# acmater/prograph

Measured on NVIDIA B200. Metric: Gpairs/s Hamming all-pairs + kNN graph build, N=1M L=256, higher is better.
Workload: dtype u8 tokens -> 5 bit planes, int32 popcount distances

## Files before the change

prograph_b200/csrc/pg_sweep.cu:

```cuda
#include <vector>
#include <mutex>

#include <cub/device/device_scan.cuh>
#include <cub/device/device_select.cuh>
#include <cub/device/device_radix_sort.cuh>
#include <thrust/iterator/counting_iterator.h>

#include <cstdlib>
#include <cmath>

#include <algorithm>

#include "pg_sweep.cuh"
#include "pg_sweep_sym.cuh"

namespace pg {

static std::mutex g_time_mu;
static bool g_time_enabled = false;
static std::vector<std::pair<cudaEvent_t, cudaEvent_t>> g_time_events;

struct SweepTimer {
  cudaEvent_t a = nullptr, b = nullptr;
  cudaStream_t s;
// ... 216 lines not shown
        const unsigned long long e = __ldcs(src + j);
        out_idx[at + j] = static_cast<long long>(e & 0xffffffffull);
        write_weight(out_w, at + j, static_cast<int>(e >> 32), weight);
      }
      at += c;
    }
  }
}

static size_t eps_counts_bytes(const Geometry& g, long long rows) { return static_cast<size_t>(g.n_splits) * rows * 8; }
static size_t eps_capture_bytes(const Geometry& g, long long rows, int cap = kEpsCapture) {
  return static_cast<size_t>(g.n_splits) * rows * static_cast<size_t>(cap) * 8;
}
static size_t eps_flag_bytes(long long rows) { return static_cast<size_t>(round_up(rows, 256)); }
static size_t eps_list_bytes(long long rows) { return static_cast<size_t>(rows) * 8; }
constexpr int kEpsCaptureMax = 1 << 20;
constexpr size_t kEpsCaptureLimit = 8ull << 30;

struct EpsPlan {
  Geometry g;
  int cap;
};
static EpsPlan eps_plan(long long rows, long long stream_rows, int words, int capture) {
  EpsPlan p;
  p.cap = 0;
  if (capture > 0 && rows < (1ll << 31)) {
    const int cap = std::min(std::max(capture, kEpsCapture), kEpsCaptureMax);
    const long long splits = static_cast<long long>(kEpsCaptureLimit / (static_cast<size_t>(rows) * cap * 8));
    if (splits >= 1) {
      p.g = make_geometry(rows, stream_rows, words, kConsumers, 0, splits);
      p.cap = cap;
      return p;
    }
  }
  p.g = make_geometry(rows, stream_rows, words, kConsumers, 0);
  if (eps_capture_bytes(p.g, rows) <= kEpsCaptureLimit && rows < (1ll << 31)) p.cap = kEpsCapture;
  return p;
}
static size_t eps_plan_bytes(const EpsPlan& p, long long rows) {
  size_t bytes = eps_counts_bytes(p.g, rows) + 256;
  if (p.cap > 0) bytes += eps_flag_bytes(rows) + eps_list_bytes(rows) + eps_capture_bytes(p.g, rows, p.cap);
  return bytes;
}


static int dispatch_sym(int planes, int words, const SymParams& prm, const SymLaunch& l, int* resident) {
#define PG_CASE(P, W) \
  if (planes == P && words == W) return sweep_sym_p##P##_w##W(prm, l, resident);
  PG_CASE(5, 1) PG_CASE(5, 2) PG_CASE(5, 4) PG_CASE(5, 8) PG_CASE(5, 16)
  PG_CASE(8, 1) PG_CASE(8, 2) PG_CASE(8, 4) PG_CASE(8, 8)
#undef PG_CASE
  set_error("symmetric sweep supports planes in {5,8} x words in {1,2,4,8} and planes=5, words=16; got planes=%d "
            "words=%d", planes, words);
  return PG_ERR_UNSUPPORTED;
}

static bool sym_shape_ok(int planes, int words) {
  return ((planes == 5 || planes == 8) && (words == 1 || words == 2 || words == 4 || words == 8)) ||
         (planes == 5 && words == 16);
}

struct SymLayout {
  int tile_cols, n_tiles, n_blocks, band_tiles, n_bands;
  size_t gnt_bytes, lock_bytes, stats_off, item_off, item_bytes_max, total;
};

static int sym_band_tiles(int tile_cols, int row_bytes) {
  double mb = 24.0;
  if (const char* ev = std::getenv("PG_SYM_BAND_MB")) mb = std::atof(ev);
  if (mb <= 0) return 1 << 30;
  long long t = static_cast<long long>(mb * 1048576.0 / (static_cast<double>(tile_cols) * row_bytes));
  if (t < 64) t = 64;
  return static_cast<int>(std::min<long long>(t, 1 << 30));
}

static SymLayout sym_layout(long long rows, int words, int planes = 5) {
  SymLayout s;
  s.tile_cols = tile_cols_for(words);
  s.n_tiles = static_cast<int>(ceil_div(rows, s.tile_cols));
  s.n_blocks = static_cast<int>(ceil_div(rows, kConsumers));
  s.band_tiles = sym_band_tiles(s.tile_cols, planes * words * 4);
  s.n_bands = static_cast<int>(ceil_div(s.n_tiles, s.band_tiles));
  s.gnt_bytes = static_cast<size_t>(round_up(static_cast<int64_t>(s.n_tiles) * s.tile_cols * 8, 256));
  s.lock_bytes = static_cast<size_t>(round_up(rows * 4, 256));
  s.stats_off = s.gnt_bytes + s.lock_bytes;
  s.item_off = s.stats_off + 256;
  const int bands8 = static_cast<int>(ceil_div(s.n_tiles, sym_band_tiles(s.tile_cols, 8 * words * 4)));
  s.item_bytes_max = (static_cast<size_t>(s.n_blocks) * (2 * static_cast<size_t>(bands8) + 2) + 64ull * 4 * 160 + 1024) *
                         sizeof(SymItem) + 8192;
  s.total = s.item_off + s.item_bytes_max;
  return s;
}

static int sym_first_tile(const SymLayout& s, int rb, long long boot_rows) {
  const long long row = static_cast<long long>(rb) * kConsumers < boot_rows ? boot_rows
                                                                            : static_cast<long long>(rb) * kConsumers;
  return static_cast<int>(row / s.tile_cols);
}

static void sym_band(const SymLayout& s, long long rows, long long boot_rows, int part, int parts, int* t0, int* t1) {
  std::vector<long long> visits(static_cast<size_t>(s.n_tiles) + 1, 0);
  for (int rb = 0; rb < s.n_blocks; ++rb) {
    const int tb = sym_first_tile(s, rb, boot_rows);
    if (tb >= s.n_tiles) continue;
    const long long in_block = std::min<long long>(kConsumers, rows - static_cast<long long>(rb) * kConsumers);
    visits[tb] += in_block;
  }
  long long total = 0, run = 0;
  for (int t = 0; t < s.n_tiles; ++t) { run += visits[t]; visits[t] = run; total += run; }
  auto bound = [&](int g) {
    if (g <= 0) return 0;
    if (g >= parts) return s.n_tiles;
    const long long want = static_cast<long long>(static_cast<double>(total) * g / parts);
    long long acc = 0;
    for (int t = 0; t < s.n_tiles; ++t) {
      acc += visits[t];
      if (acc >= want) return t + 1;
    }
    return s.n_tiles;
  };
  *t0 = bound(part);
  *t1 = bound(part + 1);
}

struct SymPlan {
  std::vector<SymItem> items;
  std::vector<int> first;
  int grid = 0;
};

static SymPlan sym_plan(const SymLayout& s, long long rows, int part, int parts, int mode, int grid,
                        long long boot_rows, int chunk_floor = 32) {
  const int boot_blocks = static_cast<int>(boot_rows / kConsumers);
  int band0 = 0, band1 = s.n_tiles;
  if (mode == 1) sym_band(s, rows, boot_rows, part, parts, &band0, &band1);
  const int rb_first = mode == 1 ? 0 : part, rb_stride = mode == 1 ? 1 : parts;
  long long total = 0;
  for (int rb = rb_first; rb < s.n_blocks; rb += rb_stride)
// ... 19 lines not shown
      const int boot = rb < boot_blocks ? 1 : 0;
      const double g = (n_seen + 0.37 * sb) * 0.6180339887498949;
      const double frac = g - static_cast<long long>(g);
      int t = tb;
      const int first = static_cast<int>(chunk / 4 + static_cast<long long>(frac * static_cast<double>(chunk))) + 1;
      while (t < te) {
        int t1 = t + (t == tb ? first : static_cast<int>(chunk));
        if (te - t1 < chunk / 4) t1 = te;
        if (t1 > te) t1 = te;
        items.push_back(SymItem{rb, t, t1, boot});
        t = t1;
      }
    }
    std::stable_sort(items.begin(), items.end(),
                     [](const SymItem& a, const SymItem& b) { return a.t1 - a.t0 > b.t1 - b.t0; });
    for (int b = 0; b < grid; ++b) heap[b] = b;
    std::make_heap(heap.begin(), heap.end(), heavier);
    for (const SymItem& it : items) {
      std::pop_heap(heap.begin(), heap.end(), heavier);
      const int b = heap.back();
      per_cta[b].push_back(it);
      load[b] += (it.t1 - it.t0) + 4;
      std::push_heap(heap.begin(), heap.end(), heavier);
    }
  }
  SymPlan plan;
  plan.first.push_back(0);
  for (int b = 0; b < grid; ++b) {
    if (per_cta[b].empty()) continue;
    plan.items.insert(plan.items.end(), per_cta[b].begin(), per_cta[b].end());
    plan.first.push_back(static_cast<int>(plan.items.size()));
  }
  plan.grid = static_cast<int>(plan.first.size()) - 1;
  return plan;
}

static int sym_knn_chunk_floor(int words, int parts) { return (parts == 1 ? 256 : 32) * std::max(1, 8 / words); }

static size_t sym_plan_bytes(const SymPlan& p) {
  return static_cast<size_t>(round_up(static_cast<int64_t>(p.first.size()) * 4, 16)) + p.items.size() * sizeof(SymItem);
}
static int sym_upload_plan(const SymPlan& p, const SymLayout& lay, char* wsb, SymParams* prm, cudaStream_t cs) {
  PG_CHECK_ARG(sym_plan_bytes(p) <= lay.item_bytes_max, "item table overflow (%zu items)", p.items.size());
  const size_t first_bytes = static_cast<size_t>(round_up(static_cast<int64_t>(p.first.size()) * 4, 16));
  PG_CUDA(cudaMemcpyAsync(wsb + lay.item_off, p.first.data(), p.first.size() * 4, cudaMemcpyHostToDevice, cs));
  PG_CUDA(cudaMemcpyAsync(wsb + lay.item_off + first_bytes, p.items.data(), p.items.size() * sizeof(SymItem),
                          cudaMemcpyHostToDevice, cs));
  prm->cta_first = reinterpret_cast<const int*>(wsb + lay.item_off);
  prm->items = reinterpret_cast<const SymItem*>(wsb + lay.item_off + first_bytes);
  prm->n_items = static_cast<int>(p.items.size());
  return PG_OK;
}

__global__ void sym_init_kernel(unsigned long long* glist, long long n_keys, unsigned long long* glast, long long n_gnt, unsigned* glock,
                                long long rows, unsigned long long* stats, int k1, int seeded) {
  if (blockIdx.x == 0 && threadIdx.x < 9) stats[threadIdx.x] = 0ull;
  const long long i = blockIdx.x * static_cast<long long>(blockDim.x) + threadIdx.x;
  const long long stride = static_cast<long long>(gridDim.x) * blockDim.x;
  if (!seeded)
    for (long long j = i; j < n_keys; j += stride) glist[j] = ~0ull;
  for (long long j = i; j < n_gnt; j += stride) {
    unsigned long long last = ~0ull;
    if (seeded && j < rows) last = glist[j * k1 + (k1 - 1)];
    glast[j] = sym_filter_word(last);
  }
  for (long long j = i; j < rows; j += stride) glock[j] = 0u;
}

__global__ void knn_part_to_lists_kernel(const unsigned long long* __restrict__ part, int n_splits, int k1,
                                         long long rows, unsigned long long* __restrict__ lists) {
  extern __shared__ unsigned long long merge_sm[];
  const long long row_base = blockIdx.x * static_cast<long long>(blockDim.x);
  const long long r = row_base + threadIdx.x;
  unsigned long long* mine = merge_sm + threadIdx.x * (k1 + 1);
  if (r < rows) {
    unsigned long long last = 0;
    bool ended = false;
    for (int j = 0; j < k1; ++j) {
      unsigned long long best = ~0ull;
      if (!ended) {
        for (int s = 0; s < n_splits; ++s) {
          const unsigned long long* lst = part + static_cast<size_t>(s) * k1 * rows + r;
          for (int i = 0; i < k1; ++i) {
            const unsigned long long v = lst[static_cast<size_t>(i) * rows];
            if (j > 0 && v <= last) continue;
            if (v < best) best = v;
            break;
          }
        }
      }
      last = best;
      ended |= best == ~0ull;
      mine[j] = best;
    }
  }
  flush_rows(merge_sm, row_base, rows, k1, PG_W_I64, true, lists, nullptr, nullptr);
}

constexpr int kMaxMergeLists = 16;

__global__ void knn_lists_finalize_kernel(const unsigned long long* __restrict__ lists, int n_lists,
                                          long long list_stride, long long row0, long long rows, int k1, int k,
                                          int drop, int weight, bool keys_out, unsigned long long* __restrict__ out_keys,
                                          long long* __restrict__ out_idx, void* out_w) {
  extern __shared__ unsigned long long merge_sm[];
  const long long row_base = blockIdx.x * static_cast<long long>(blockDim.x);
  const long long r = row_base + threadIdx.x;
  unsigned long long* mine = merge_sm + threadIdx.x * (k + 1);
  if (r < rows) {
    const unsigned long long* base = lists + static_cast<size_t>(row0 + r) * k1;
    unsigned long long head[kMaxMergeLists];
    int pos[kMaxMergeLists];
#pragma unroll
    for (int s = 0; s < kMaxMergeLists; ++s) {
      pos[s] = 0;
      head[s] = s < n_lists ? base[static_cast<size_t>(s) * list_stride] : ~0ull;
    }
    for (int j = 0; j < drop + k; ++j) {
      unsigned long long best = ~0ull;
// ... 359 lines not shown
  }
  if (rc != PG_OK) return rc;
  const int threads = rows_per_merge_block(k1);
  knn_part_to_lists_kernel<<<static_cast<unsigned>(ceil_div(rows, threads)), threads, merge_smem_bytes(k1), l.stream>>>(
      prm.part, g.n_splits, k1, rows, reinterpret_cast<unsigned long long*>(lists));
  PG_LAUNCH_CHECK();
  return PG_OK;
}

int pg_knn_sym_band(int64_t rows, int words, int64_t boot_rows, int part, int parts, int64_t* row_begin,
                    int64_t* row_end) {
  PG_CHECK_ARG(rows > 0 && words > 0 && parts >= 1 && part >= 0 && part < parts && row_begin && row_end,
               "bad band arguments");
  const SymLayout lay = sym_layout(rows, words);
  int t0 = 0, t1 = 0;
  sym_band(lay, rows, boot_rows, part, parts, &t0, &t1);
  *row_begin = std::min<int64_t>(rows, static_cast<int64_t>(t0) * lay.tile_cols);
  *row_end = std::min<int64_t>(rows, static_cast<int64_t>(t1) * lay.tile_cols);
  return PG_OK;
}

int pg_knn_sym_plan(int64_t rows, int planes, int words, int64_t boot_rows, int part, int parts, int mode, int grid,
                    int32_t* items_host, int64_t capacity, int64_t* n_items) {
  PG_CHECK_ARG(rows > 0 && words > 0 && planes > 0 && parts >= 1 && part >= 0 && part < parts && grid >= 1 && n_items &&
                   (mode == 0 || mode == 1) && boot_rows >= 0 && boot_rows % kStreamRowPad == 0,
               "bad plan arguments");
  const SymLayout lay = sym_layout(rows, words, planes);
  const SymPlan plan = sym_plan(lay, rows, part, parts, mode, grid, boot_rows, sym_knn_chunk_floor(words, parts));
  *n_items = static_cast<int64_t>(plan.items.size());
  PG_CHECK_ARG(sym_plan_bytes(plan) <= lay.item_bytes_max, "item table overflow (%zu items)", plan.items.size());
  if (items_host) {
    int cta = 0;
    for (size_t i = 0; i < plan.items.size() && static_cast<int64_t>(i) < capacity; ++i) {
      while (static_cast<int>(i) >= plan.first[cta + 1]) ++cta;
      items_host[5 * i + 0] = plan.items[i].rb;
      items_host[5 * i + 1] = plan.items[i].t0;
      items_host[5 * i + 2] = plan.items[i].t1;
      items_host[5 * i + 3] = plan.items[i].boot;
      items_host[5 * i + 4] = cta;
    }
  }
  return PG_OK;
}

int pg_knn_sym_status(const void* workspace, int64_t rows, int words, void* stream) {
  PG_CHECK_ARG(workspace && rows > 0 && words > 0, "bad status arguments");
  const SymLayout lay = sym_layout(rows, words);
  unsigned err = 0;
  cudaStream_t cs = static_cast<cudaStream_t>(stream);
  PG_CUDA(cudaMemcpyAsync(&err, static_cast<const char*>(workspace) + lay.stats_off + 64, sizeof(err),
                          cudaMemcpyDeviceToHost, cs));
  PG_CUDA(cudaStreamSynchronize(cs));
  if (err != 0) {
    set_error("symmetric sweep: a row lock could not be taken within %u attempts (lists are incomplete)", kLockSpinLimit);
    return PG_ERR_CUDA;
  }
  return PG_OK;
}

int pg_hamming_knn_sym(const uint32_t* table, int64_t rows, int planes, int words, int k1, int part, int parts,
                       int mode, int64_t boot_rows, uint64_t* lists, void* workspace, size_t workspace_bytes,
                       void* stream) {
  const int rb_first = part, rb_stride = parts;
  PG_CHECK_ARG(mode == 0 || mode == 1, "bad partition mode %d", mode);
  PG_CHECK_ARG(table && lists && workspace, "null pointer");
  PG_CHECK_ARG(rows > 0 && rows < (1ll << 31), "row count out of range");
  PG_CHECK_ARG((reinterpret_cast<uintptr_t>(table) & 15) == 0, "table must be 16-byte aligned");
  PG_CHECK_ARG((reinterpret_cast<uintptr_t>(workspace) & 255) == 0, "workspace must be 256-byte aligned");
  PG_CHECK_ARG(rb_stride >= 1 && rb_first >= 0 && rb_first < rb_stride, "bad row-block interleave %d/%d", rb_first,
               rb_stride);
  PG_CHECK_ARG(boot_rows >= 0 && boot_rows % kStreamRowPad == 0 && boot_rows <= rows,
               "bootstrap rows must be a multiple of %d within the table", kStreamRowPad);
  if (!sym_shape_ok(planes, words) || k1 < 1 || k1 > 32) {
    set_error("symmetric sweep: planes/words %d/%d or list length %d not covered", planes, words, k1);
    return PG_ERR_UNSUPPORTED;
  }
  const SymLayout lay = sym_layout(rows, words, planes);
  PG_CHECK_ARG(workspace_bytes >= lay.total, "workspace too small: %zu < %zu", workspace_bytes, lay.total);
  cudaStream_t cs = static_cast<cudaStream_t>(stream);
  char* wsb = static_cast<char*>(workspace);
  SymParams prm;
  memset(&prm, 0, sizeof(prm));
  prm.tab = table;
  prm.rows = rows;
  prm.one = 1u;
  prm.k1 = k1;
  prm.boot_rows = boot_rows;
  prm.glist = reinterpret_cast<unsigned long long*>(lists);
  prm.glast = reinterpret_cast<unsigned long long*>(wsb);
  prm.glock = reinterpret_cast<unsigned*>(wsb + lay.gnt_bytes);
  unsigned long long* stats_dev = reinterpret_cast<unsigned long long*>(wsb + lay.stats_off);
  const bool want_stats = std::getenv("PG_SYM_STATS") != nullptr;
  prm.stats = want_stats ? stats_dev : nullptr;
  prm.error = reinterpret_cast<unsigned*>(stats_dev + 8);
  SymLaunch l{0, static_cast<size_t>(k1) * kConsumers * 8, cs, SYM_KNN};
  int resident = 0;
  int rc = dispatch_sym(planes, words, prm, l, &resident);
  if (rc != PG_OK) return rc;
  const SymPlan plan = sym_plan(lay, rows, part, parts, mode, resident, boot_rows, sym_knn_chunk_floor(words, parts));
  sym_init_kernel<<<num_sms() * 4, 256, 0, cs>>>(prm.glist, static_cast<long long>(rows) * k1, prm.glast,
                                                 static_cast<long long>(lay.n_tiles) * lay.tile_cols, prm.glock, rows,
                                                 stats_dev, k1, boot_rows > 0 ? 1 : 0);
  PG_LAUNCH_CHECK();
  if (plan.items.empty()) return PG_OK;
  rc = sym_upload_plan(plan, lay, wsb, &prm, cs);
  if (rc != PG_OK) return rc;
  l.grid = plan.grid;
  {
    SweepTimer t(cs);
    rc = dispatch_sym(planes, words, prm, l, nullptr);
  }
  if (rc == PG_OK && want_stats) {
    unsigned long long st[8];
    PG_CUDA(cudaMemcpyAsync(st, stats_dev, sizeof(st), cudaMemcpyDeviceToHost, cs));
    PG_CUDA(cudaStreamSynchronize(cs));
    fprintf(stderr, "[pg sym] rows=%lld boot=%lld items=%d grid=%d | locks %llu, lock spins %llu, list writes %llu | row "
            "inserts %llu\n", static_cast<long long>(rows), static_cast<long long>(boot_rows), prm.n_items, l.grid,
            st[1], st[2], st[3], st[4]);
  }
  return rc;
}

int pg_hamming_eps_sym(const uint32_t* table, int64_t rows, int planes, int words, const uint32_t* lut_host,
                       int lut_words, int part, int parts, int mode, uint64_t* keys, int64_t capacity,
                       uint64_t* counters, void* workspace, size_t workspace_bytes, void* stream) {
  PG_CHECK_ARG(table && keys && counters && workspace && lut_host, "null pointer");
  PG_CHECK_ARG(rows > 0 && rows < (1ll << 27), "row count out of range for packed edge keys");
  PG_CHECK_ARG((reinterpret_cast<uintptr_t>(table) & 15) == 0, "table must be 16-byte aligned");
  PG_CHECK_ARG((reinterpret_cast<uintptr_t>(workspace) & 255) == 0, "workspace must be 256-byte aligned");
  PG_CHECK_ARG(parts >= 1 && part >= 0 && part < parts && (mode == 0 || mode == 1), "bad partition %d/%d mode %d", part,
               parts, mode);
  PG_CHECK_ARG(lut_words >= 1 && lut_words <= kMaxLutWords && lut_words * 32 > words * 32, "lut must cover distances 0..%d",
               words * 32);
  PG_CHECK_ARG(capacity >= 0, "negative capacity");
  if (!sym_shape_ok(planes, words)) {
    set_error("symmetric sweep: planes/words %d/%d not covered", planes, words);
    return PG_ERR_UNSUPPORTED;
  }
  SymParams prm;
  memset(&prm, 0, sizeof(prm));
  unsigned span = 0;
  if (!lut_as_range(lut_host, lut_words, &prm.lo, &span)) {
    set_error("symmetric epsilon sweep needs a contiguous distance range");
    return PG_ERR_UNSUPPORTED;
  }
  prm.hi = prm.lo == 0x7fffffff ? -1 : prm.lo + static_cast<int>(span);
  if (prm.lo == 0x7fffffff) prm.lo = 1 << 20;
  const SymLayout lay = sym_layout(rows, words, planes);
  PG_CHECK_ARG(workspace_bytes >= lay.total, "workspace too small: %zu < %zu", workspace_bytes, lay.total);
  const EdgeKeyBits kb = edge_key_bits(rows, words);
  cudaStream_t cs = static_cast<cudaStream_t>(stream);
  char* wsb = static_cast<char*>(workspace);
  prm.tab = table;
  prm.rows = rows;
  prm.one = 1u;
  prm.k1 = 1;
  prm.sh_col = kb.dbits;
  prm.sh_row = kb.dbits + kb.idxbits;
  prm.keys = reinterpret_cast<unsigned long long*>(keys);
  prm.capacity = capacity;
  prm.counters = reinterpret_cast<unsigned long long*>(counters);
  SymLaunch l{0, 0, cs, SYM_EPS};
  int resident = 0;
  int rc = dispatch_sym(planes, words, prm, l, &resident);
  if (rc != PG_OK) return rc;
  const SymPlan plan = sym_plan(lay, rows, part, parts, mode, resident, 0);
  PG_CUDA(cudaMemsetAsync(counters, 0, 2 * sizeof(uint64_t), cs));
  if (plan.items.empty()) return PG_OK;
  rc = sym_upload_plan(plan, lay, wsb, &prm, cs);
// ... 148 lines not shown
```

prograph_b200/csrc/pg_sweep_inst.cu:

```cuda
#include "pg_sweep.cuh"
#include "pg_sweep_sym.cuh"

#ifndef PG_P
#error "compile with -DPG_P=<planes> -DPG_W=<words>"
#endif

#define PG_CAT2(a, b, c, d) a##b##c##d
#define PG_NAME(P, W) PG_CAT2(sweep_p, P, _w, W)

namespace pg {
int PG_NAME(PG_P, PG_W)(const SweepParams& prm, const SweepLaunch& l) { return launch_sweep<PG_P, PG_W>(prm, l); }
#define PG_SYM_NAME(P, W) PG_CAT2(sweep_sym_p, P, _w, W)
int PG_SYM_NAME(PG_P, PG_W)(const SymParams& prm, const SymLaunch& l, int* resident) {
  return launch_sweep_sym<PG_P, PG_W>(prm, l, resident);
}
}
```

prograph_b200/csrc/pg_sweep_sym.cuh:

```cuda
#pragma once
#include "pg_sweep.cuh"

namespace pg {

constexpr int kTauInf = 0x3fffffff;

struct SymItem { int rb, t0, t1, boot; };

struct SymParams {
  const uint32_t* tab;
  long long rows;
  const SymItem* items;
  const int* cta_first;
  int n_items;
  unsigned one;
  int k1;
  unsigned long long* glist;
  unsigned long long* glast;
  unsigned* glock;
  unsigned long long* stats;
  unsigned* error;
  long long boot_rows;
  int lo, hi;
  int sh_row, sh_col;
  unsigned long long* keys;
  long long capacity;
  unsigned long long* counters;
};

__device__ __forceinline__ unsigned long long ld_cg_u64(const unsigned long long* p) {
  unsigned long long v;
  asm volatile("ld.global.cg.u64 %0, [%1];" : "=l"(v) : "l"(p) : "memory");
  return v;
}
__device__ __forceinline__ void st_cg_u64(unsigned long long* p, unsigned long long v) {
  asm volatile("st.global.cg.u64 [%0], %1;" ::"l"(p), "l"(v) : "memory");
}
__device__ __forceinline__ unsigned atom_cas_acquire_gpu(unsigned* p, unsigned cmp, unsigned val) {
  unsigned old;
  asm volatile("atom.acquire.gpu.global.cas.b32 %0, [%1], %2, %3;" : "=r"(old) : "l"(p), "r"(cmp), "r"(val) : "memory");
  return old;
}
__device__ __forceinline__ void st_release_gpu_u32(unsigned* p, unsigned v) {
  asm volatile("st.release.gpu.global.u32 [%0], %1;" ::"l"(p), "r"(v) : "memory");
}
constexpr unsigned kLockSpinLimit = 1u << 24;
__host__ __device__ __forceinline__ unsigned long long sym_filter_word(unsigned long long last) {
  const unsigned tau = (last == ~0ull) ? static_cast<unsigned>(kTauInf) : static_cast<unsigned>(last >> 32);
  return (static_cast<unsigned long long>(~tau) << 32) | (last & 0xffffffffull);
}
__device__ __forceinline__ int mad_s32(int a, unsigned b, int c) {
  int r;
  asm("mad.lo.s32 %0, %1, %2, %3;" : "=r"(r) : "r"(a), "r"(b), "r"(c));
  return r;
}

static __device__ __noinline__ void sym_serve_col(const SymParams& prm, long long j, unsigned long long key, bool is_cand,
                                           int lane) {
  const int k1 = prm.k1;
  unsigned long long* lst = prm.glist + static_cast<size_t>(j) * k1;
  unsigned cand = __ballot_sync(0xffffffffu, is_cand);
  if (cand == 0u) return;
  unsigned* lock = prm.glock + j;
  unsigned got = 1u;
  if (lane == 0) {
    unsigned spins = 0;
    while (atom_cas_acquire_gpu(lock, 0u, 1u) != 0u) {
      __nanosleep(100);
      if (++spins > kLockSpinLimit) {
        got = 0u;
        atomicExch(prm.error, 1u);
        break;
      }
    }
    if (prm.stats != nullptr) {
      atomicAdd(prm.stats + 1, 1ull);
      if (spins) atomicAdd(prm.stats + 2, static_cast<unsigned long long>(spins));
    }
  }
  if (__shfl_sync(0xffffffffu, got, 0) == 0u) return;
  __syncwarp();
  unsigned long long e = lane < k1 ? ld_cg_u64(lst + lane) : ~0ull;
  bool changed = false;
  while (cand) {
    const int src = __ffs(cand) - 1;
    cand &= cand - 1;
    const unsigned long long kk = __shfl_sync(0xffffffffu, key, src);
    const int pos = __popc(__ballot_sync(0xffffffffu, lane < k1 && e < kk));
    const unsigned long long up = __shfl_up_sync(0xffffffffu, e, 1);
    if (pos < k1) {
      if (lane == pos) e = kk;
      else if (lane > pos) e = up;
      changed = true;
    }
  }
  if (changed) {
    if (lane < k1) st_cg_u64(lst + lane, e);
    const unsigned long long last = __shfl_sync(0xffffffffu, e, k1 - 1);
    if (lane == 0) {
      st_cg_u64(prm.glast + j, sym_filter_word(last));
      if (prm.stats != nullptr) atomicAdd(prm.stats + 3, 1ull);
    }
  }
  __syncwarp();
  if (lane == 0) st_release_gpu_u32(lock, 0u);
}

constexpr int kMaxSymList = 32;

static __device__ __noinline__ int sym_serve_row(unsigned long long* warp_lists, int k1, unsigned cand, unsigned dv,
                                          unsigned col, int lane, int tau_seed, int tau,
                                          unsigned long long* stats) {
  if (stats != nullptr && lane == 0) atomicAdd(stats + 4, static_cast<unsigned long long>(__popc(cand)));
  while (cand) {
    const int src = __ffs(cand) - 1;
    cand &= cand - 1;
    const unsigned dd = __shfl_sync(0xffffffffu, dv, src);
    const unsigned long long key = (static_cast<unsigned long long>(dd) << 32) | col;
    const unsigned t_new = knn_insert_coop(warp_lists + static_cast<size_t>(src) * k1, k1, key, lane);
    if (lane == src) tau = min(tau_seed, t_new == 0xffffffffu ? kTauInf : static_cast<int>(t_new));
  }
  return tau;
}

struct SymCursor {
  int idx, end, t, t1;
  __device__ __forceinline__ void start(int i, const SymParams& prm) {
    idx = i;
    if (idx < end) {
      const int4 it = __ldg(reinterpret_cast<const int4*>(prm.items) + idx);
      t = it.y;
      t1 = it.z;
    } else {
      t = t1 = 0;
    }
  }
  __device__ __forceinline__ bool valid() const { return idx < end; }
  __device__ __forceinline__ void advance(const SymParams& prm) {
    if (++t == t1) start(idx + 1, prm);
  }
};

enum SymMode { SYM_KNN = 0, SYM_EPS = 1 };

constexpr int kEdgeChunk = 512;

static __device__ __noinline__ void sym_emit(const SymParams& prm, bool hit, unsigned long long key_fwd,
                                             unsigned long long key_rev, bool both, int lane, long long& ch_base,
                                             int& ch_used, unsigned long long& n_real) {
  const unsigned m = __ballot_sync(0xffffffffu, hit);
  if (m == 0u) return;
  const int mult = both ? 2 : 1;
  const int n = __popc(m) * mult;
  if (ch_base == -1 || ch_used + n > kEdgeChunk) {
    if (ch_base >= 0)
      for (int sl = ch_used + lane; sl < kEdgeChunk; sl += 32) prm.keys[ch_base + sl] = ~0ull;
    unsigned long long b = 0;
    if (lane == 0) b = atomicAdd(prm.counters, static_cast<unsigned long long>(kEdgeChunk));
// ... 181 lines not shown
        }
      }
      if (la.valid()) la.advance(prm);
      if (++stage == kStages) { stage = 0; phase ^= 1u; }
    }

    if constexpr (MODE == SYM_KNN) {
      __syncwarp();
      const long long wrow0 = static_cast<long long>(rb) * kConsumers + (warp << 5);
#pragma unroll 1
      for (int src = 0; src < 32; ++src) {
        if (wrow0 + src >= prm.rows) break;
        const unsigned long long lk = lane < k1 ? warp_lists[static_cast<size_t>(src) * k1 + lane] : ~0ull;
        sym_serve_col(prm, wrow0 + src, lk, lk != ~0ull, lane);
      }
      __syncwarp();
    }
  }
  if constexpr (MODE == SYM_EPS) {
    if (ch_base >= 0)
      for (int sl = ch_used + lane; sl < kEdgeChunk; sl += 32) prm.keys[ch_base + sl] = ~0ull;
    if (lane == 0 && n_real) atomicAdd(prm.counters + 1, n_real);
  }
}

struct SymLaunch {
  int grid;
  size_t list_bytes;
  cudaStream_t stream;
  int mode = SYM_KNN;
};


template <int P, int W, int MODE>
int launch_sweep_sym_mode(const SymParams& prm, const SymLaunch& l, int* resident) {
  auto kern = sweep_sym_kernel<P, W, MODE>;
  const size_t smem = static_cast<size_t>(kStages) * (TileCols<W>::value * P * W * 4 +
                                                      (MODE == SYM_KNN ? TileCols<W>::value * 8 : 0)) +
                      2 * kStages * sizeof(uint64_t) + l.list_bytes;
  PG_CUDA(cudaFuncSetAttribute(kern, cudaFuncAttributeMaxDynamicSharedMemorySize, static_cast<int>(smem)));
  int occ = 0;
  PG_CUDA(cudaOccupancyMaxActiveBlocksPerMultiprocessor(&occ, kern, kSweepThreads, smem));
  if (occ < 1) { set_error("symmetric sweep does not fit on an SM (smem %zu bytes)", smem); return PG_ERR_UNSUPPORTED; }
  if (resident) *resident = num_sms() * occ;
  if (l.grid <= 0) return PG_OK;
  kern<<<static_cast<unsigned>(l.grid), kSweepThreads, smem, l.stream>>>(prm);
  PG_LAUNCH_CHECK();
  return PG_OK;
}

template <int P, int W>
int launch_sweep_sym(const SymParams& prm, const SymLaunch& l, int* resident) {
  if (l.mode == SYM_EPS) return launch_sweep_sym_mode<P, W, SYM_EPS>(prm, l, resident);
  return launch_sweep_sym_mode<P, W, SYM_KNN>(prm, l, resident);
}

#define PG_DECL_SWEEP_SYM(P, W) int sweep_sym_p##P##_w##W(const SymParams& prm, const SymLaunch& l, int* resident);
PG_DECL_SWEEP_SYM(5, 1) PG_DECL_SWEEP_SYM(5, 2) PG_DECL_SWEEP_SYM(5, 4) PG_DECL_SWEEP_SYM(5, 8) PG_DECL_SWEEP_SYM(5, 16)
PG_DECL_SWEEP_SYM(8, 1) PG_DECL_SWEEP_SYM(8, 2) PG_DECL_SWEEP_SYM(8, 4) PG_DECL_SWEEP_SYM(8, 8)
#undef PG_DECL_SWEEP_SYM

}
```

Measured before the change: 655.9.

## Add one-hot symbol-match sweep for 5-plane symmetric kNN

For planes=5 with up to 8 words, the symmetric kNN sweep now first builds a one-hot layout of the column tiles. For each 32-column tile and each position, it stores one word per symbol with one bit per column that holds that symbol. Each row's query tokens then index shared memory directly to fetch match masks. A carry-save adder tree built from lop3 counts matches per column in bit-sliced form, and a bit-sliced compare against thresholds replaces per-pair XOR and popcount across planes. This adds a max-token scan with a host sync, a temporary buffer allocation, and a layout kernel inside the timed region, which costs extra memory traffic.

Measured after the change: 1108 (median of 6 runs). 1.69x the previous value.

```diff
diff --git a/prograph_b200/csrc/pg_sweep.cu b/prograph_b200/csrc/pg_sweep.cu
--- a/prograph_b200/csrc/pg_sweep.cu
+++ b/prograph_b200/csrc/pg_sweep.cu
@@ -292,6 +292,17 @@
 #undef PG_CASE
   set_error("symmetric sweep supports planes in {5,8} x words in {1,2,4,8} and planes=5, words=16; got planes=%d "
             "words=%d", planes, words);
+  return PG_ERR_UNSUPPORTED;
+}
+
+static bool sym_onehot_shape(int planes, int words) { return planes == 5 && words <= 8; }
+
+static int dispatch_sym_onehot(int words, const SymParams& prm, const SymLaunch& l, int symbols, int* resident) {
+  if (words == 1) return sweep_sym_onehot_w1(prm, l, symbols, resident);
+  if (words == 2) return sweep_sym_onehot_w2(prm, l, symbols, resident);
+  if (words == 4) return sweep_sym_onehot_w4(prm, l, symbols, resident);
+  if (words == 8) return sweep_sym_onehot_w8(prm, l, symbols, resident);
+  set_error("one-hot symmetric sweep: words=%d not covered", words);
   return PG_ERR_UNSUPPORTED;
 }
 
@@ -462,6 +473,52 @@
     glast[j] = sym_filter_word(last);
   }
   for (long long j = i; j < rows; j += stride) glock[j] = 0u;
+}
+
+__global__ void sym_max_token_kernel(const uint32_t* __restrict__ tab, long long rows, int words, int* __restrict__ out) {
+  const long long n = rows * words;
+  int best = 0;
+  for (long long e = blockIdx.x * static_cast<long long>(blockDim.x) + threadIdx.x; e < n;
+       e += static_cast<long long>(gridDim.x) * blockDim.x) {
+    const long long row = e / words;
+    const int w = static_cast<int>(e - row * words);
+    const uint32_t* src = tab + static_cast<size_t>(row) * 5 * words + w;
+    uint32_t cand = 0xffffffffu;
+    int mx = 0;
+    for (int p = 4; p >= 0; --p) {
+      const uint32_t x = __ldg(src + p * words) & cand;
+      if (x) { mx |= 1 << p; cand = x; }
+    }
+    best = max(best, mx);
+  }
+  best = static_cast<int>(__reduce_max_sync(0xffffffffu, static_cast<unsigned>(best)));
+  if ((threadIdx.x & 31) == 0 && best > 0) atomicMax(out, best);
+}
+
+__global__ void __launch_bounds__(256) sym_onehot_kernel(const uint32_t* __restrict__ tab, long long n_st, int words,
+                                                         int S, uint32_t* __restrict__ out) {
+  const int lane = threadIdx.x & 31;
+  const long long n_warps = n_st * words;
+  for (long long gw = (blockIdx.x * static_cast<long long>(blockDim.x) + threadIdx.x) >> 5; gw < n_warps;
+       gw += (static_cast<long long>(gridDim.x) * blockDim.x) >> 5) {
+    const long long t = gw / words;
+    const int w = static_cast<int>(gw - t * words);
+    const uint32_t* src = tab + static_cast<size_t>(t * 32 + lane) * 5 * words + w;
+    uint32_t x[5];
+#pragma unroll
+    for (int p = 0; p < 5; ++p) x[p] = __ldg(src + p * words);
+    uint32_t flip[5];
+#pragma unroll
+    for (int p = 0; p < 5; ++p) flip[p] = ((lane >> p) & 1) ? 0u : 0xffffffffu;
+    uint32_t* dst = out + (static_cast<size_t>(t) * 32 * words + static_cast<size_t>(w) * 32) * S;
+#pragma unroll 4
+    for (int j = 0; j < 32; ++j) {
+      uint32_t e = 0xffffffffu;
+#pragma unroll
+      for (int p = 0; p < 5; ++p) e &= __ballot_sync(0xffffffffu, (x[p] >> j) & 1u) ^ flip[p];
+      if (lane < S) dst[static_cast<size_t>(j) * S + lane] = e;
+    }
+  }
 }
 
 __global__ void knn_part_to_lists_kernel(const unsigned long long* __restrict__ part, int n_splits, int k1,
@@ -969,8 +1026,23 @@
   prm.stats = want_stats ? stats_dev : nullptr;
   prm.error = reinterpret_cast<unsigned*>(stats_dev + 8);
   SymLaunch l{0, static_cast<size_t>(k1) * kConsumers * 8, cs, SYM_KNN};
+  const bool onehot = sym_onehot_shape(planes, words);
+  int symbols = 0;
+  if (onehot) {
+    int* max_dev = reinterpret_cast<int*>(stats_dev + 16);
+    int max_token = 0;
+    PG_CUDA(cudaMemsetAsync(max_dev, 0, sizeof(int), cs));
+    sym_max_token_kernel<<<num_sms() * 4, 256, 0, cs>>>(table, rows, words, max_dev);
+    PG_LAUNCH_CHECK();
+    PG_CUDA(cudaMemcpyAsync(&max_token, max_dev, sizeof(int), cudaMemcpyDeviceToHost, cs));
+    PG_CUDA(cudaStreamSynchronize(cs));
+    symbols = onehot_symbols(max_token);
+  }
+  auto run = [&](int* res) {
+    return onehot ? dispatch_sym_onehot(words, prm, l, symbols, res) : dispatch_sym(planes, words, prm, l, res);
+  };
   int resident = 0;
-  int rc = dispatch_sym(planes, words, prm, l, &resident);
+  int rc = run(&resident);
   if (rc != PG_OK) return rc;
   const SymPlan plan = sym_plan(lay, rows, part, parts, mode, resident, boot_rows, sym_knn_chunk_floor(words, parts));
   sym_init_kernel<<<num_sms() * 4, 256, 0, cs>>>(prm.glist, static_cast<long long>(rows) * k1, prm.glast,
@@ -981,10 +1053,27 @@
   rc = sym_upload_plan(plan, lay, wsb, &prm, cs);
   if (rc != PG_OK) return rc;
   l.grid = plan.grid;
+  void* onehot_buf = nullptr;
+  if (onehot) {
+    const long long n_st = ceil_div(rows, kOnehotRows);
+    PG_CUDA(temp_alloc(&onehot_buf, static_cast<size_t>(n_st) * 32 * words * symbols * 4, cs));
+    prm.onehot = static_cast<const uint32_t*>(onehot_buf);
+  }
   {
     SweepTimer t(cs);
-    rc = dispatch_sym(planes, words, prm, l, nullptr);
-  }
+    if (onehot) {
+      const long long n_warps = ceil_div(rows, kOnehotRows) * words;
+      sym_onehot_kernel<<<static_cast<unsigned>(std::min<long long>(ceil_div(n_warps, 8), num_sms() * 16ll)), 256, 0,
+                          cs>>>(table, ceil_div(rows, kOnehotRows), words, symbols,
+                                static_cast<uint32_t*>(onehot_buf));
+      count_launch();
+      const cudaError_t e = cudaGetLastError();
+      rc = e == cudaSuccess ? PG_OK : PG_ERR_CUDA;
+      if (e != cudaSuccess) set_error("one-hot layout launch failed: %s", cudaGetErrorString(e));
+    }
+    if (rc == PG_OK) rc = run(nullptr);
+  }
+  if (onehot_buf) cudaFreeAsync(onehot_buf, cs);
   if (rc == PG_OK && want_stats) {
     unsigned long long st[8];
     PG_CUDA(cudaMemcpyAsync(st, stats_dev, sizeof(st), cudaMemcpyDeviceToHost, cs));
diff --git a/prograph_b200/csrc/pg_sweep_inst.cu b/prograph_b200/csrc/pg_sweep_inst.cu
--- a/prograph_b200/csrc/pg_sweep_inst.cu
+++ b/prograph_b200/csrc/pg_sweep_inst.cu
@@ -14,4 +14,11 @@
 int PG_SYM_NAME(PG_P, PG_W)(const SymParams& prm, const SymLaunch& l, int* resident) {
   return launch_sweep_sym<PG_P, PG_W>(prm, l, resident);
 }
+#if PG_P == 5 && PG_W <= 8
+#define PG_CAT3(a, b) a##b
+#define PG_ONEHOT_NAME(W) PG_CAT3(sweep_sym_onehot_w, W)
+int PG_ONEHOT_NAME(PG_W)(const SymParams& prm, const SymLaunch& l, int symbols, int* resident) {
+  return launch_sweep_sym_onehot<PG_W>(prm, l, symbols, resident);
 }
+#endif
+}
diff --git a/prograph_b200/csrc/pg_sweep_sym.cuh b/prograph_b200/csrc/pg_sweep_sym.cuh
--- a/prograph_b200/csrc/pg_sweep_sym.cuh
+++ b/prograph_b200/csrc/pg_sweep_sym.cuh
@@ -9,6 +9,7 @@
 
 struct SymParams {
   const uint32_t* tab;
+  const uint32_t* onehot;
   long long rows;
   const SymItem* items;
   const int* cta_first;
@@ -391,7 +392,12 @@
 template <int P, int W>
 int launch_sweep_sym(const SymParams& prm, const SymLaunch& l, int* resident) {
   if (l.mode == SYM_EPS) return launch_sweep_sym_mode<P, W, SYM_EPS>(prm, l, resident);
-  return launch_sweep_sym_mode<P, W, SYM_KNN>(prm, l, resident);
+  if constexpr (P == 5 && W <= 8) {
+    set_error("symmetric kNN of planes=5, words=%d runs on the one-hot sweep", W);
+    return PG_ERR_UNSUPPORTED;
+  } else {
+    return launch_sweep_sym_mode<P, W, SYM_KNN>(prm, l, resident);
+  }
 }
 
 #define PG_DECL_SWEEP_SYM(P, W) int sweep_sym_p##P##_w##W(const SymParams& prm, const SymLaunch& l, int* resident);
@@ -399,4 +405,270 @@
 PG_DECL_SWEEP_SYM(8, 1) PG_DECL_SWEEP_SYM(8, 2) PG_DECL_SWEEP_SYM(8, 4) PG_DECL_SWEEP_SYM(8, 8)
 #undef PG_DECL_SWEEP_SYM
 
-}
+constexpr int kOnehotRows = 32;
+constexpr int kOnehotMaxStages = 16;
+
+__device__ __forceinline__ uint32_t lop_xor3(uint32_t a, uint32_t b, uint32_t c) {
+  uint32_t r;
+  asm("lop3.b32 %0, %1, %2, %3, 0x96;" : "=r"(r) : "r"(a), "r"(b), "r"(c));
+  return r;
+}
+__device__ __forceinline__ uint32_t lop_maj3(uint32_t a, uint32_t b, uint32_t c) {
+  uint32_t r;
+  asm("lop3.b32 %0, %1, %2, %3, 0xE8;" : "=r"(r) : "r"(a), "r"(b), "r"(c));
+  return r;
+}
+
+template <int S, int POS>
+__device__ __forceinline__ uint32_t onehot_match(const uint32_t* q, uint32_t base) {
+  const uint32_t a = __byte_perm(q[POS / 4], base, 0x7650u | (POS % 4));
+  uint32_t v;
+  asm volatile("ld.shared.u32 %0, [%1+%2];" : "=r"(v) : "r"(a), "n"(POS * S * 4));
+  return v;
+}
+
+template <int S, int K, int BASE>
+__device__ __forceinline__ uint32_t onehot_tree(uint32_t (&acc)[9], const uint32_t* q, uint32_t base) {
+  uint32_t a, b;
+  if constexpr (K == 1) {
+    a = onehot_match<S, BASE>(q, base);
+    b = onehot_match<S, BASE + 1>(q, base);
+  } else {
+    a = onehot_tree<S, K - 1, BASE>(acc, q, base);
+    b = onehot_tree<S, K - 1, BASE + (1 << (K - 1))>(acc, q, base);
+  }
+  const uint32_t carry = lop_maj3(acc[K - 1], a, b);
+  acc[K - 1] = lop_xor3(acc[K - 1], a, b);
+  return carry;
+}
+
+__device__ __forceinline__ uint32_t onehot_ge512(const uint32_t (&m)[9], const uint32_t (&kb)[9]) {
+  uint32_t c = m[0] & kb[0];
+#pragma unroll
+  for (int i = 1; i < 9; ++i) c = lop_maj3(m[i], kb[i], c);
+  return c;
+}
+
+template <int W, int S>
+__global__ void __launch_bounds__(kSweepThreads, 2) sweep_sym_onehot_kernel(const __grid_constant__ SymParams prm,
+                                                                            const int nst) {
+  constexpr int NPOS = 32 * W;
+  constexpr int LOGN = W == 1 ? 5 : (W == 2 ? 6 : (W == 4 ? 7 : 8));
+  static_assert((1 << LOGN) == NPOS && S <= 32, "one-hot sweep: rows of 32, 64, 128 or 256 positions, tokens < 32");
+  constexpr uint32_t STAGE_BYTES = NPOS * S * 4;
+  constexpr uint32_t STAGE_STRIDE = (STAGE_BYTES + 255) / 256 * 256;
+  constexpr uint32_t TAU_BYTES = kOnehotRows * 8;
+  constexpr int R = TileCols<W>::value / kOnehotRows;
+
+  extern __shared__ __align__(128) unsigned char smem_raw[];
+  const uint32_t raw_u32 = smem_u32(smem_raw);
+  unsigned char* sm = smem_raw + (((raw_u32 + 255u) & ~255u) - raw_u32);
+  const uint32_t stage_u32 = smem_u32(sm);
+  unsigned long long* taus = reinterpret_cast<unsigned long long*>(sm + nst * STAGE_STRIDE);
+  uint64_t* full = reinterpret_cast<uint64_t*>(sm + nst * (STAGE_STRIDE + TAU_BYTES));
+  unsigned* done = reinterpret_cast<unsigned*>(full + kOnehotMaxStages);
+  unsigned long long* lists = reinterpret_cast<unsigned long long*>(full + 2 * kOnehotMaxStages);
+
+  const int tid = threadIdx.x;
+  const int warp = tid >> 5;
+  const int lane = tid & 31;
+  const int k1 = prm.k1;
+  unsigned long long* warp_lists = lists + static_cast<size_t>(warp << 5) * k1;
+  const int n_st = static_cast<int>(ceil_div(prm.rows, kOnehotRows));
+
+  auto fill_stage = [&](int s, int t) {
+    mbar_arrive_expect_tx(&full[s], STAGE_BYTES + TAU_BYTES);
+    bulk_g2s(sm + s * STAGE_STRIDE, prm.onehot + static_cast<size_t>(t) * (NPOS * S), STAGE_BYTES, &full[s]);
+    bulk_g2s(taus + s * kOnehotRows, prm.glast + static_cast<size_t>(t) * kOnehotRows, TAU_BYTES, &full[s]);
+  };
+  int la_idx = 0, la_t = 0, la_t1 = 0;
+  const int item_first = __ldg(prm.cta_first + blockIdx.x), item_end = __ldg(prm.cta_first + blockIdx.x + 1);
+  auto la_start = [&](int i) {
+    la_idx = i;
+    if (i < item_end) {
+      const int4 it = __ldg(reinterpret_cast<const int4*>(prm.items) + i);
+      la_t = it.y * R;
+      la_t1 = min(it.z * R, n_st);
+    }
+  };
+  auto la_advance = [&]() {
+    if (++la_t == la_t1) la_start(la_idx + 1);
+  };
+  la_start(item_first);
+  if (tid == 0) {
+    for (int s = 0; s < nst; ++s) {
+      mbar_init(&full[s], 1);
+      done[s] = 0;
+    }
+    fence_mbar_init();
+  }
+  __syncthreads();
+#pragma unroll 1
+  for (int s = 0; s < nst; ++s) {
+    if (tid == 0 && la_idx < item_end) fill_stage(s, la_t);
+    if (la_idx < item_end) la_advance();
+  }
+
+  int stage = 0;
+  uint32_t phase = 0;
+
+  for (int ii = item_first; ii < item_end; ++ii) {
+    const int4 it = __ldg(reinterpret_cast<const int4*>(prm.items) + ii);
+    const int rb = it.x;
+    const int t0 = it.y * R, t1 = min(it.z * R, n_st);
+    const bool boot = it.w != 0;
+    const int r = rb * kConsumers + tid;
+    const bool valid = r < prm.rows;
+    uint32_t q[NPOS / 4];
+    {
+      const uint32_t* src = prm.tab + static_cast<size_t>(valid ? r : 0) * (5 * W);
+#pragma unroll
+      for (int w = 0; w < W; ++w) {
+        uint32_t x[5];
+#pragma unroll
+        for (int p = 0; p < 5; ++p) x[p] = valid ? __ldg(src + p * W + w) : 0u;
+#pragma unroll
+        for (int g = 0; g < 8; ++g) {
+          uint32_t v = 0;
+#pragma unroll
+          for (int p = 0; p < 5; ++p) v |= ((((x[p] >> (4 * g)) & 0xfu) * 0x00204081u) & 0x01010101u) << (p + 2);
+          q[8 * w + g] = v;
+        }
+      }
+    }
+    int tau_seed = 0, tau = 0;
+    if (valid) {
+      const int g = ~static_cast<int>(ld_cg_u64(prm.glast + r) >> 32);
+      tau_seed = g >= kTauInf ? kTauInf : g + 1;
+    }
+    tau = tau_seed;
+    for (int j = lane; j < 32 * k1; j += 32) warp_lists[j] = ~0ull;
+    const unsigned vmask = (valid && !boot) ? 0xffffffffu : 0u;
+    const int diag_begin = boot ? static_cast<int>(prm.boot_rows) : rb * kConsumers;
+    const int diag_end = boot ? 0x7fffffff : diag_begin + kConsumers;
+    __syncwarp();
+
+    for (int t = t0; t < t1; ++t) {
+      mbar_wait(&full[stage], phase);
+      const uint32_t base = stage_u32 + stage * STAGE_STRIDE;
+      const unsigned long long* tnt = taus + stage * kOnehotRows;
+      const int col0 = t * kOnehotRows;
+      const int ncols = min(kOnehotRows, static_cast<int>(prm.rows) - col0);
+      const int c = min(ncols, max(0, diag_begin - col0));
+      const int c_mid = min(ncols, max(c, diag_end - col0));
+
+      uint32_t m[9];
+#pragma unroll
+      for (int i = 0; i < 9; ++i) m[i] = 0u;
+      m[LOGN] = onehot_tree<S, LOGN, 0>(m, q, base);
+
+      const unsigned below_end = ncols >= 32 ? 0xffffffffu : ~(0xffffffffu << ncols);
+      const unsigned row_on = c >= 32 ? 0u : (0xffffffffu << c) & below_end;
+      const unsigned col_on = c_mid >= 32 ? 0u : (0xffffffffu << c_mid) & below_end & vmask;
+      uint32_t kb[9];
+      unsigned cand = 0u;
+      if (c_mid < ncols && !boot) {
+        const int tj = ~static_cast<int>(tnt[lane] >> 32);
+        const int kc = 511 - (NPOS - 1 - min(tj, NPOS));
+#pragma unroll
+        for (int i = 0; i < 9; ++i) kb[i] = __ballot_sync(0xffffffffu, (kc >> i) & 1);
+        const unsigned pass = __ballot_sync(0xffffffffu, tj >= NPOS);
+        cand = (onehot_ge512(m, kb) | pass) & col_on;
+      }
+      {
+        const int kr = 511 - NPOS + min(tau, NPOS + 1);
+#pragma unroll
+        for (int i = 0; i < 9; ++i) kb[i] = 0u - ((static_cast<unsigned>(kr) >> i) & 1u);
+        const unsigned pass = tau > NPOS ? 0xffffffffu : 0u;
+        cand |= (onehot_ge512(m, kb) | pass) & row_on;
+      }
+
+      if (__any_sync(0xffffffffu, cand != 0u)) {
+        unsigned todo = __reduce_or_sync(0xffffffffu, cand);
+        while (todo) {
+          const int b = __ffs(todo) - 1;
+          todo &= todo - 1;
+          int mb = 0;
+#pragma unroll
+          for (int i = 0; i < 9; ++i) mb |= static_cast<int>((m[i] >> b) & 1u) << i;
+          const int dv = NPOS - mb;
+          const unsigned col = static_cast<unsigned>(col0 + b);
+          const unsigned rc = __ballot_sync(0xffffffffu, dv < tau);
+          if (rc) tau = sym_serve_row(warp_lists, k1, rc, static_cast<unsigned>(dv), col, lane, tau_seed, tau, prm.stats);
+          if (b >= c_mid) {
+            const unsigned long long fw = tnt[b];
+            const unsigned long long lastk = (static_cast<unsigned long long>(~static_cast<unsigned>(fw >> 32)) << 32) |
+                                             (fw & 0xffffffffull);
+            const unsigned long long mine = (static_cast<unsigned long long>(static_cast<unsigned>(dv)) << 32) |
+                                            static_cast<unsigned>(r);
+            const bool cc = vmask != 0u && mine < lastk;
+            if (__any_sync(0xffffffffu, cc)) sym_serve_col(prm, col, mine, cc, lane);
+          }
+        }
+      }
+
+      __syncwarp();
+      if (lane == 0) {
+        if (atom_add_acq_rel_cta(&done[stage], 1u) == kConsumerWarps - 1) {
+          done[stage] = 0;
+          if (la_idx < item_end) {
+            fence_proxy_async();
+            fill_stage(stage, la_t);
+          }
+        }
+      }
+      if (la_idx < item_end) la_advance();
+      if (++stage == nst) { stage = 0; phase ^= 1u; }
+    }
+
+    __syncwarp();
+    const long long wrow0 = static_cast<long long>(rb) * kConsumers + (warp << 5);
+#pragma unroll 1
+    for (int src = 0; src < 32; ++src) {
+      if (wrow0 + src >= prm.rows) break;
+      const unsigned long long lk = lane < k1 ? warp_lists[static_cast<size_t>(src) * k1 + lane] : ~0ull;
+      sym_serve_col(prm, wrow0 + src, lk, lk != ~0ull, lane);
+    }
+    __syncwarp();
+  }
+}
+
+template <int W, int S>
+size_t onehot_smem_bytes(int nst, size_t list_bytes) {
+  const size_t stage = (static_cast<size_t>(32 * W * S * 4) + 255) / 256 * 256 + kOnehotRows * 8;
+  return 256 + static_cast<size_t>(nst) * stage + 2 * kOnehotMaxStages * sizeof(uint64_t) + list_bytes;
+}
+
+template <int W, int S>
+int launch_sweep_sym_onehot_s(const SymParams& prm, const SymLaunch& l, int* resident) {
+  auto kern = sweep_sym_onehot_kernel<W, S>;
+  int nst = 24 / W < kOnehotMaxStages ? 24 / W : kOnehotMaxStages, occ = 0;
+  size_t smem = 0;
+  for (;; --nst) {
+    smem = onehot_smem_bytes<W, S>(nst, l.list_bytes);
+    PG_CUDA(cudaFuncSetAttribute(kern, cudaFuncAttributeMaxDynamicSharedMemorySize, static_cast<int>(smem)));
+    PG_CUDA(cudaOccupancyMaxActiveBlocksPerMultiprocessor(&occ, kern, kSweepThreads, smem));
+    if (occ >= 2 || nst == 2) break;
+  }
+  if (occ < 1) { set_error("symmetric one-hot sweep does not fit on an SM (smem %zu bytes)", smem); return PG_ERR_UNSUPPORTED; }
+  if (resident) *resident = num_sms() * occ;
+  if (l.grid <= 0) return PG_OK;
+  kern<<<static_cast<unsigned>(l.grid), kSweepThreads, smem, l.stream>>>(prm, nst);
+  PG_LAUNCH_CHECK();
+  return PG_OK;
+}
+
+inline int onehot_symbols(int max_token) { return max_token <= 20 ? 21 : 32; }
+
+template <int W>
+int launch_sweep_sym_onehot(const SymParams& prm, const SymLaunch& l, int symbols, int* resident) {
+  if (symbols == 21) return launch_sweep_sym_onehot_s<W, 21>(prm, l, resident);
+  return launch_sweep_sym_onehot_s<W, 32>(prm, l, resident);
+}
+
+#define PG_DECL_SWEEP_ONEHOT(W) \
+  int sweep_sym_onehot_w##W(const SymParams& prm, const SymLaunch& l, int symbols, int* resident);
+PG_DECL_SWEEP_ONEHOT(1) PG_DECL_SWEEP_ONEHOT(2) PG_DECL_SWEEP_ONEHOT(4) PG_DECL_SWEEP_ONEHOT(8)
+#undef PG_DECL_SWEEP_ONEHOT
+
+}
```

## Replace per-row spin locks with lock-free CAS replace-max list insertion

Applied to the files above, without the earlier changes.

Column-side kNN list updates no longer take a per-row spin lock with nanosleep backoff. Each warp now swaps the current maximum entry of an unsorted list using atomicCAS, retrying on conflict. The lists are left unsorted during the sweep, so a warp bitonic sort kernel runs afterwards and the seeded init takes the max over the whole list. This removes lock acquire/release traffic and contention, at the cost of an extra sort pass and CAS retries under contention.

Measured after the change: 654.3 before, 655.7 after (median of 6 runs). No clear change (+0.2%).

```diff
diff --git a/prograph_b200/csrc/pg_sweep.cu b/prograph_b200/csrc/pg_sweep.cu
--- a/prograph_b200/csrc/pg_sweep.cu
+++ b/prograph_b200/csrc/pg_sweep.cu
@@ -302,7 +302,7 @@
 
 struct SymLayout {
   int tile_cols, n_tiles, n_blocks, band_tiles, n_bands;
-  size_t gnt_bytes, lock_bytes, stats_off, item_off, item_bytes_max, total;
+  size_t gnt_bytes, stats_off, item_off, item_bytes_max, total;
 };
 
 static int sym_band_tiles(int tile_cols, int row_bytes) {
@@ -322,8 +322,7 @@
   s.band_tiles = sym_band_tiles(s.tile_cols, planes * words * 4);
   s.n_bands = static_cast<int>(ceil_div(s.n_tiles, s.band_tiles));
   s.gnt_bytes = static_cast<size_t>(round_up(static_cast<int64_t>(s.n_tiles) * s.tile_cols * 8, 256));
-  s.lock_bytes = static_cast<size_t>(round_up(rows * 4, 256));
-  s.stats_off = s.gnt_bytes + s.lock_bytes;
+  s.stats_off = s.gnt_bytes;
   s.item_off = s.stats_off + 256;
   const int bands8 = static_cast<int>(ceil_div(s.n_tiles, sym_band_tiles(s.tile_cols, 8 * words * 4)));
   s.item_bytes_max = (static_cast<size_t>(s.n_blocks) * (2 * static_cast<size_t>(bands8) + 2) + 64ull * 4 * 160 + 1024) *
@@ -449,7 +448,7 @@
   return PG_OK;
 }
 
-__global__ void sym_init_kernel(unsigned long long* glist, long long n_keys, unsigned long long* glast, long long n_gnt, unsigned* glock,
+__global__ void sym_init_kernel(unsigned long long* glist, long long n_keys, unsigned long long* glast, long long n_gnt,
                                 long long rows, unsigned long long* stats, int k1, int seeded) {
   if (blockIdx.x == 0 && threadIdx.x < 9) stats[threadIdx.x] = 0ull;
   const long long i = blockIdx.x * static_cast<long long>(blockDim.x) + threadIdx.x;
@@ -458,10 +457,31 @@
     for (long long j = i; j < n_keys; j += stride) glist[j] = ~0ull;
   for (long long j = i; j < n_gnt; j += stride) {
     unsigned long long last = ~0ull;
-    if (seeded && j < rows) last = glist[j * k1 + (k1 - 1)];
+    if (seeded && j < rows) {
+      last = 0ull;
+      for (int s = 0; s < k1; ++s) last = max(last, glist[j * k1 + s]);
+    }
     glast[j] = sym_filter_word(last);
   }
-  for (long long j = i; j < rows; j += stride) glock[j] = 0u;
+}
+
+__global__ void sym_sort_lists_kernel(unsigned long long* lists, long long rows, int k1) {
+  const int lane = threadIdx.x & 31;
+  const long long warps = static_cast<long long>(gridDim.x) * (blockDim.x >> 5);
+  for (long long r = blockIdx.x * static_cast<long long>(blockDim.x >> 5) + (threadIdx.x >> 5); r < rows; r += warps) {
+    unsigned long long* lst = lists + static_cast<size_t>(r) * k1;
+    unsigned long long v = lane < k1 ? lst[lane] : ~0ull;
+#pragma unroll
+    for (int size = 2; size <= 32; size <<= 1) {
+#pragma unroll
+      for (int stride = size >> 1; stride > 0; stride >>= 1) {
+        const unsigned long long o = __shfl_xor_sync(0xffffffffu, v, stride);
+        const bool keep_min = ((lane & stride) == 0) == ((lane & size) == 0);
+        v = keep_min ? min(v, o) : max(v, o);
+      }
+    }
+    if (lane < k1) lst[lane] = v;
+  }
 }
 
 __global__ void knn_part_to_lists_kernel(const unsigned long long* __restrict__ part, int n_splits, int k1,
@@ -927,7 +947,8 @@
                           cudaMemcpyDeviceToHost, cs));
   PG_CUDA(cudaStreamSynchronize(cs));
   if (err != 0) {
-    set_error("symmetric sweep: a row lock could not be taken within %u attempts (lists are incomplete)", kLockSpinLimit);
+    set_error("symmetric sweep: a list insertion failed %u compare-and-swaps in a row (lists are incomplete)",
+              kCasRetryLimit);
     return PG_ERR_CUDA;
   }
   return PG_OK;
@@ -963,7 +984,6 @@
   prm.boot_rows = boot_rows;
   prm.glist = reinterpret_cast<unsigned long long*>(lists);
   prm.glast = reinterpret_cast<unsigned long long*>(wsb);
-  prm.glock = reinterpret_cast<unsigned*>(wsb + lay.gnt_bytes);
   unsigned long long* stats_dev = reinterpret_cast<unsigned long long*>(wsb + lay.stats_off);
   const bool want_stats = std::getenv("PG_SYM_STATS") != nullptr;
   prm.stats = want_stats ? stats_dev : nullptr;
@@ -974,8 +994,8 @@
   if (rc != PG_OK) return rc;
   const SymPlan plan = sym_plan(lay, rows, part, parts, mode, resident, boot_rows, sym_knn_chunk_floor(words, parts));
   sym_init_kernel<<<num_sms() * 4, 256, 0, cs>>>(prm.glist, static_cast<long long>(rows) * k1, prm.glast,
-                                                 static_cast<long long>(lay.n_tiles) * lay.tile_cols, prm.glock, rows,
-                                                 stats_dev, k1, boot_rows > 0 ? 1 : 0);
+                                                 static_cast<long long>(lay.n_tiles) * lay.tile_cols, rows, stats_dev, k1,
+                                                 boot_rows > 0 ? 1 : 0);
   PG_LAUNCH_CHECK();
   if (plan.items.empty()) return PG_OK;
   rc = sym_upload_plan(plan, lay, wsb, &prm, cs);
@@ -985,11 +1005,16 @@
     SweepTimer t(cs);
     rc = dispatch_sym(planes, words, prm, l, nullptr);
   }
+  if (rc == PG_OK && std::getenv("PG_SYM_UNSORTED") == nullptr) {
+    sym_sort_lists_kernel<<<static_cast<unsigned>(std::min<long long>(ceil_div(rows, 8), num_sms() * 16ll)), 256, 0, cs>>>(
+        prm.glist, rows, k1);
+    PG_LAUNCH_CHECK();
+  }
   if (rc == PG_OK && want_stats) {
     unsigned long long st[8];
     PG_CUDA(cudaMemcpyAsync(st, stats_dev, sizeof(st), cudaMemcpyDeviceToHost, cs));
     PG_CUDA(cudaStreamSynchronize(cs));
-    fprintf(stderr, "[pg sym] rows=%lld boot=%lld items=%d grid=%d | locks %llu, lock spins %llu, list writes %llu | row "
+    fprintf(stderr, "[pg sym] rows=%lld boot=%lld items=%d grid=%d | CAS %llu, CAS failed %llu, list writes %llu | row "
             "inserts %llu\n", static_cast<long long>(rows), static_cast<long long>(boot_rows), prm.n_items, l.grid,
             st[1], st[2], st[3], st[4]);
   }
diff --git a/prograph_b200/csrc/pg_sweep_sym.cuh b/prograph_b200/csrc/pg_sweep_sym.cuh
--- a/prograph_b200/csrc/pg_sweep_sym.cuh
+++ b/prograph_b200/csrc/pg_sweep_sym.cuh
@@ -17,7 +17,6 @@
   int k1;
   unsigned long long* glist;
   unsigned long long* glast;
-  unsigned* glock;
   unsigned long long* stats;
   unsigned* error;
   long long boot_rows;
@@ -36,15 +35,7 @@
 __device__ __forceinline__ void st_cg_u64(unsigned long long* p, unsigned long long v) {
   asm volatile("st.global.cg.u64 [%0], %1;" ::"l"(p), "l"(v) : "memory");
 }
-__device__ __forceinline__ unsigned atom_cas_acquire_gpu(unsigned* p, unsigned cmp, unsigned val) {
-  unsigned old;
-  asm volatile("atom.acquire.gpu.global.cas.b32 %0, [%1], %2, %3;" : "=r"(old) : "l"(p), "r"(cmp), "r"(val) : "memory");
-  return old;
-}
-__device__ __forceinline__ void st_release_gpu_u32(unsigned* p, unsigned v) {
-  asm volatile("st.release.gpu.global.u32 [%0], %1;" ::"l"(p), "r"(v) : "memory");
-}
-constexpr unsigned kLockSpinLimit = 1u << 24;
+constexpr unsigned kCasRetryLimit = 1u << 24;
 __host__ __device__ __forceinline__ unsigned long long sym_filter_word(unsigned long long last) {
   const unsigned tau = (last == ~0ull) ? static_cast<unsigned>(kTauInf) : static_cast<unsigned>(last >> 32);
   return (static_cast<unsigned long long>(~tau) << 32) | (last & 0xffffffffull);
@@ -53,6 +44,17 @@
   int r;
   asm("mad.lo.s32 %0, %1, %2, %3;" : "=r"(r) : "r"(a), "r"(b), "r"(c));
   return r;
+}
+
+__device__ __forceinline__ unsigned long long warp_max_u64(unsigned long long v) {
+  const unsigned hi = __reduce_max_sync(0xffffffffu, static_cast<unsigned>(v >> 32));
+  const unsigned lo = __reduce_max_sync(0xffffffffu, static_cast<unsigned>(v >> 32) == hi ? static_cast<unsigned>(v) : 0u);
+  return (static_cast<unsigned long long>(hi) << 32) | lo;
+}
+__device__ __forceinline__ unsigned long long warp_min_u64(unsigned long long v) {
+  const unsigned hi = __reduce_min_sync(0xffffffffu, static_cast<unsigned>(v >> 32));
+  const unsigned lo = __reduce_min_sync(0xffffffffu, static_cast<unsigned>(v >> 32) == hi ? static_cast<unsigned>(v) : ~0u);
+  return (static_cast<unsigned long long>(hi) << 32) | lo;
 }
 
 static __device__ __noinline__ void sym_serve_col(const SymParams& prm, long long j, unsigned long long key, bool is_cand,
@@ -61,49 +63,36 @@
   unsigned long long* lst = prm.glist + static_cast<size_t>(j) * k1;
   unsigned cand = __ballot_sync(0xffffffffu, is_cand);
   if (cand == 0u) return;
-  unsigned* lock = prm.glock + j;
-  unsigned got = 1u;
-  if (lane == 0) {
-    unsigned spins = 0;
-    while (atom_cas_acquire_gpu(lock, 0u, 1u) != 0u) {
-      __nanosleep(100);
-      if (++spins > kLockSpinLimit) {
-        got = 0u;
-        atomicExch(prm.error, 1u);
-        break;
-      }
-    }
-    if (prm.stats != nullptr) {
-      atomicAdd(prm.stats + 1, 1ull);
-      if (spins) atomicAdd(prm.stats + 2, static_cast<unsigned long long>(spins));
-    }
-  }
-  if (__shfl_sync(0xffffffffu, got, 0) == 0u) return;
-  __syncwarp();
-  unsigned long long e = lane < k1 ? ld_cg_u64(lst + lane) : ~0ull;
-  bool changed = false;
+  unsigned long long e = lane < k1 ? ld_cg_u64(lst + lane) : 0ull;
+  unsigned long long mx = warp_max_u64(e);
+  unsigned attempts = 0, fails = 0;
   while (cand) {
-    const int src = __ffs(cand) - 1;
-    cand &= cand - 1;
-    const unsigned long long kk = __shfl_sync(0xffffffffu, key, src);
-    const int pos = __popc(__ballot_sync(0xffffffffu, lane < k1 && e < kk));
-    const unsigned long long up = __shfl_up_sync(0xffffffffu, e, 1);
-    if (pos < k1) {
-      if (lane == pos) e = kk;
-      else if (lane > pos) e = up;
-      changed = true;
-    }
-  }
-  if (changed) {
-    if (lane < k1) st_cg_u64(lst + lane, e);
-    const unsigned long long last = __shfl_sync(0xffffffffu, e, k1 - 1);
-    if (lane == 0) {
-      st_cg_u64(prm.glast + j, sym_filter_word(last));
-      if (prm.stats != nullptr) atomicAdd(prm.stats + 3, 1ull);
-    }
-  }
-  __syncwarp();
-  if (lane == 0) st_release_gpu_u32(lock, 0u);
+    const unsigned long long kk = warp_min_u64((cand >> lane) & 1u ? key : ~0ull);
+    cand &= ~__ballot_sync(0xffffffffu, (cand >> lane) & 1u && key == kk);
+    while (kk < mx) {
+      const int slot = __ffs(__ballot_sync(0xffffffffu, lane < k1 && e == mx)) - 1;
+      unsigned long long old = 0;
+      if (lane == slot) {
+        old = atomicCAS(lst + slot, mx, kk);
+        e = old == mx ? kk : old;
+      }
+      old = __shfl_sync(0xffffffffu, old, slot);
+      ++attempts;
+      const bool won = old == mx;
+      mx = warp_max_u64(e);
+      if (won) break;
+      if (++fails > kCasRetryLimit) {
+        if (lane == 0) atomicExch(prm.error, 1u);
+        return;
+      }
+    }
+  }
+  if (attempts > fails && lane == 0) st_cg_u64(prm.glast + j, sym_filter_word(mx));
+  if (prm.stats != nullptr && lane == 0 && attempts) {
+    atomicAdd(prm.stats + 1, static_cast<unsigned long long>(attempts));
+    if (fails) atomicAdd(prm.stats + 2, static_cast<unsigned long long>(fails));
+    if (attempts > fails) atomicAdd(prm.stats + 3, 1ull);
+  }
 }
 
 constexpr int kMaxSymList = 32;
```
